# CrispyChillies/Image-Retrieval---Thesis-2026

Hardware: AMD Instinct MI355X
Metric: queries/sec (embed+top-10) over 1M x 1024 gallery (higher is better)
Workload: dtype f32 embed (two fp16 MFMA terms); bf16 MFMA candidates + f64 re-rank

## Files before the change

image-retrieval---thesis-2026_amd/csrc/k_conv3x3_d2h.hip:

```cpp
#include "mirx_kernels.h"

namespace mirx {

namespace {

typedef __attribute__((ext_vector_type(8))) _Float16 f16x8;
typedef __attribute__((ext_vector_type(16))) float f32x16;
typedef __attribute__((ext_vector_type(4))) unsigned u32x4;
typedef __attribute__((ext_vector_type(2))) float f32x2;
typedef __attribute__((ext_vector_type(2))) _Float16 f16x2;

#define LDS_PTR(p) ((__attribute__((address_space(3))) void *)(p))

constexpr int CIN = 128, COUT = 32;
constexpr int KC = 16;
constexpr int NST = CIN / KC;

template <int W, int R, int IPW = 1, int NW = 4>
__global__ __launch_bounds__(64 * NW, NW == 8 ? 1 : 2) void k_conv3x3_d2p(const uint16_t *__restrict__ yt, const uint16_t *__restrict__ w3,
                                                        const float *__restrict__ oscale, float *__restrict__ out,
                                                        int64_t out_bs, const float *__restrict__ in_inv,
                                                        unsigned *__restrict__ out_range, int64_t out_ps, int64_t n_img,
                                                        const float *__restrict__ pool_sc, const float *__restrict__ pool_sh,
                                                        float *__restrict__ pool_out, int64_t pool_bs) {
    constexpr int PW = W + 2, PR = R + 2;
    static_assert(IPW == 1 || R == W, "several images per workgroup: whole images only");
    constexpr int NPIX = IPW * PR * PW;
    constexpr int NP = (NPIX + 31) / 32;
    constexpr int PLANE = NP * 32 * 32;
    constexpr int STAGE = 2 * PLANE;
    constexpr int WSTAGE = 9 * 2 * COUT * KC * 2;
    constexpr int W_LDS0 = 2 * STAGE;
    constexpr int NOUT = IPW * R * W;
    constexpr int NBLK = (NOUT + 31) / 32;
    static_assert(NBLK <= 2 * NW, "two column blocks per wave");
    constexpr int PPW = (2 * NP + NW - 1) / NW;
    constexpr int WPW = (18 + NW - 1) / NW;
    extern __shared__ __attribute__((aligned(16))) char sm[];

    const int wave = __builtin_amdgcn_readfirstlane(threadIdx.x >> 6), lane = threadIdx.x & 63;
    const int half = lane >> 5, n = lane & 31;
    int strip = blockIdx.x;
    int64_t img = blockIdx.y;
    {
        const unsigned nstrip = gridDim.x, lin = blockIdx.x + nstrip * blockIdx.y, full = gridDim.y & ~7u;
        if (lin < nstrip * full) {
            const unsigned j = lin >> 3;
            strip = (int)(j % nstrip);
            img = (int64_t)(j / nstrip) * 8 + (lin & 7);
        }
    }
    const int oy0 = strip * R;
    constexpr unsigned IMG_BYTES = 16u * W * W * 32u;
    img *= IPW;
    const int n_here = (int)(n_img - img < IPW ? n_img - img : IPW);
    const __amdgpu_buffer_rsrc_t yrsrc = __builtin_amdgcn_make_buffer_rsrc((void *)(yt + img * (int64_t)(IMG_BYTES / 2)), 0,
                                                                           (unsigned)n_here * IMG_BYTES, 0x00020000);
    unsigned a_src[PPW];
    int a_dst[PPW];
#pragma unroll
    for (int i = 0; i < PPW; ++i) {
        const int q = wave + NW * i;
        const int term = q / NP, piece = q % NP;
        const int pix = piece * 32 + (lane >> 1);
        const int ji = pix / (PR * PW), prem = pix % (PR * PW);
        const int pr = prem / PW, pc = prem % PW;
        const int iy = oy0 - 1 + pr, ix = pc - 1;
        const bool inside = q < 2 * NP && pix < NPIX && iy >= 0 && iy < W && ix >= 0 && ix < W;
        const int chunk = (lane & 1) ^ ((pix >> 3) & 1);
        a_src[i] = inside ? (unsigned)(ji * IMG_BYTES + (term * W * W + iy * W + ix) * 32 + chunk * 16) : 0xfffffff0u;
        a_dst[i] = q < 2 * NP ? term * PLANE + piece * 1024 : -1;
    }
    auto dma_a = [&](int st, int buf) {
#pragma unroll
        for (int i = 0; i < PPW; ++i)
            if (a_dst[i] >= 0) {
                const unsigned v = a_src[i] == 0xfffffff0u ? a_src[i] : a_src[i] + (unsigned)st * (2u * W * W * 32u);
                __builtin_amdgcn_raw_ptr_buffer_load_lds(yrsrc, LDS_PTR(sm + buf * STAGE + a_dst[i]), 16, v, 0, 0, 0);
            }
    };

    int pbase[2];
    bool live_blk[2];
#pragma unroll
    for (int t = 0; t < 2; ++t) {
        const int blk = wave + NW * t;
        live_blk[t] = blk < NBLK;
        int p = blk * 32 + n;
        if (p >= NOUT) p = NOUT - 1;
        const int pj = p / (R * W), pq = p % (R * W);
        pbase[t] = pj * (PR * PW) + (pq / W) * PW + (pq % W);
    }
    const int a_off = n * 32 + ((half ^ ((n >> 3) & 1)) << 4);
    const __amdgpu_buffer_rsrc_t wrsrc = __builtin_amdgcn_make_buffer_rsrc((void *)w3, 0, NST * WSTAGE, 0x00020000);
    const int w_voff = (lane >> 1) * 32 + (((lane & 1) ^ ((lane >> 4) & 1)) << 4);
    auto dma_w = [&](int st, int buf) {
#pragma unroll
        for (int i = 0; i < WPW; ++i) {
            const int piece = wave + NW * i;
            if (piece < 18)
                __builtin_amdgcn_raw_ptr_buffer_load_lds(wrsrc, LDS_PTR(sm + W_LDS0 + buf * WSTAGE + piece * 1024), 16, w_voff,
                                                         st * WSTAGE + piece * 1024, 0, 0);
        }
    };

    f32x16 acc[2];
#pragma unroll
    for (int t = 0; t < 2; ++t)
#pragma unroll
        for (int r = 0; r < 16; ++r) acc[t][r] = 0.f;

#define MIRX_D2P_READA(DST, TAP)                                                                   \
    {                                                                                              \
        DST[0] = *reinterpret_cast<const f16x8 *>(wb + (2 * (TAP)) * 1024 + a_off);                \
        DST[1] = *reinterpret_cast<const f16x8 *>(wb + (2 * (TAP) + 1) * 1024 + a_off);            \
    }
#define MIRX_D2P_READB(DST, TAP, T)                                                                \
    {                                                                                              \
        const int pix_ = pbase[T] + ((TAP) / 3) * PW + (TAP) % 3;                                  \
        const char *pb_ = sb + pix_ * 32 + ((half ^ ((pix_ >> 3) & 1)) << 4);                      \
        DST[0] = *reinterpret_cast<const f16x8 *>(pb_);                                            \
        DST[1] = *reinterpret_cast<const f16x8 *>(pb_ + PLANE);                                    \
    }
#define MIRX_D2P_MFMA(T, A, B)                                                                     \
    {                                                                                              \
        f32x16 c_ = acc[T];                                                                        \
        c_ = __builtin_amdgcn_mfma_f32_32x32x16_f16(A[1], B[0], c_, 0, 0, 0);                      \
        c_ = __builtin_amdgcn_mfma_f32_32x32x16_f16(A[0], B[1], c_, 0, 0, 0);                      \
        c_ = __builtin_amdgcn_mfma_f32_32x32x16_f16(A[0], B[0], c_, 0, 0, 0);                      \
        acc[T] = c_;                                                                               \
    }
    const bool two = live_blk[1];
    dma_w(0, 0);
    dma_a(0, 0);
    for (int st = 0; st < NST; ++st) {
        const int cur = st & 1;
        asm volatile("s_waitcnt vmcnt(0)" ::: "memory");
        __syncthreads();
        if (st + 1 < NST) {
            dma_w(st + 1, cur ^ 1);
            dma_a(st + 1, cur ^ 1);
        }
        __builtin_amdgcn_sched_barrier(0);
        const char *sb = sm + cur * STAGE;
        const char *wb = sm + W_LDS0 + cur * WSTAGE;
        f16x8 a0[2], a1[2], b0[2], b1[2];
        MIRX_D2P_READA(a0, 0)
        MIRX_D2P_READB(b0, 0, 0)
        if (two) {
#pragma unroll
            for (int tap = 0; tap < 9; ++tap) {
                MIRX_D2P_READB(b1, tap, 1)
                if (tap + 1 < 9) {
                    if (tap & 1) { MIRX_D2P_READA(a0, tap + 1) } else { MIRX_D2P_READA(a1, tap + 1) }
                }
                __builtin_amdgcn_sched_barrier(0);
                if (tap & 1) { MIRX_D2P_MFMA(0, a1, b0) } else { MIRX_D2P_MFMA(0, a0, b0) }
                if (tap + 1 < 9) MIRX_D2P_READB(b0, tap + 1, 0)
                __builtin_amdgcn_sched_barrier(0);
                if (tap & 1) { MIRX_D2P_MFMA(1, a1, b1) } else { MIRX_D2P_MFMA(1, a0, b1) }
            }
        } else {
#pragma unroll
            for (int tap = 0; tap < 9; ++tap) {
                if (tap + 1 < 9) {
                    MIRX_D2P_READB(b1, tap + 1, 0)
                    if (tap & 1) { MIRX_D2P_READA(a0, tap + 1) } else { MIRX_D2P_READA(a1, tap + 1) }
                }
                __builtin_amdgcn_sched_barrier(0);
                if (tap & 1) { MIRX_D2P_MFMA(0, a1, b0) } else { MIRX_D2P_MFMA(0, a0, b0) }
#pragma unroll
                for (int q = 0; q < 2; ++q) b0[q] = b1[q];
            }
        }
    }
#undef MIRX_D2P_READA
#undef MIRX_D2P_READB
#undef MIRX_D2P_MFMA

    float *oi = out + img * out_bs + (int64_t)oy0 * W;
    float osc[16];
#pragma unroll
    for (int r = 0; r < 16; ++r) osc[r] = oscale[8 * (r >> 2) + (r & 3) + 4 * half];
    constexpr int ACT_PITCH = NOUT + 1;
    float *s_act = reinterpret_cast<float *>(sm);
    const bool pooled_twin = IPW == 1 && pool_out != nullptr;
    float psc[16], psh[16];
    if (pooled_twin) {
#pragma unroll
        for (int r = 0; r < 16; ++r) {
            psc[r] = pool_sc[8 * (r >> 2) + (r & 3) + 4 * half];
            psh[r] = pool_sh[8 * (r >> 2) + (r & 3) + 4 * half];
        }
        __syncthreads();
    }
#pragma unroll
    for (int t = 0; t < 2; ++t) {
        const int p = (wave + NW * t) * 32 + n;
        const int pj = p / (R * W), pq = p % (R * W);
        const bool live = live_blk[t] && p < NOUT && pj < n_here && oy0 + pq / W < W;
        const int pimg = (int)img + (pj < n_here ? pj : 0);
        float vmax = 0.f;
        if (live) {
            const float x_inv = in_inv[pimg];
            float *op = oi + (int64_t)pj * out_bs + pq;
#pragma unroll
            for (int r = 0; r < 16; ++r) {
                const int oc = 8 * (r >> 2) + (r & 3) + 4 * half;
                const float v = acc[t][r] * (osc[r] * x_inv);
                vmax = range_max(vmax, v);
                op[(int64_t)oc * out_ps] = v;
                if (pooled_twin) s_act[oc * ACT_PITCH + p] = fmaxf(fmaf(v, psc[r], psh[r]), 0.0f);
            }
        }
        if (out_range && live_blk[t]) {
            if (IPW == 1) range_publish(out_range, (int)img, vmax, lane);
            else range_publish_lanes(out_range, pimg, vmax, lane);
        }
    }
    if constexpr (IPW == 1) {
        if (pooled_twin) {
            __syncthreads();
            constexpr int W2 = W / 2, R2 = R / 2, NP2 = R2 * W2;
            static_assert(R % 2 == 0 && W % 2 == 0, "whole row pairs");
            const int rows_here = W - oy0 < R ? W - oy0 : R;
            float *po = pool_out + img * pool_bs + (int64_t)(oy0 / 2) * W2;
            for (int i = threadIdx.x; i < COUT * NP2; i += 64 * NW) {
                const int oc = i / NP2, q = i % NP2, py = q / W2, px = q % W2;
                if (2 * py < rows_here) {
                    const float *a = s_act + oc * ACT_PITCH + (2 * py) * W + 2 * px;
                    po[(int64_t)oc * (W2 * W2) + q] = (a[0] + a[1] + a[W] + a[W + 1]) * 0.25f;
                }
            }
        }
    }
}

template <int W, int R, int IPW = 1, int NW = 4>
hipError_t launch_d2p(const uint16_t *yt, const uint16_t *w2, const float *oscale, int64_t n, float *out, int64_t out_bs,
                      const float *in_inv, float *out_range, int64_t out_ps, hipStream_t st, const float *pool_sc = nullptr,
                      const float *pool_sh = nullptr, float *pool_out = nullptr, int64_t pool_bs = 0) {
    constexpr int NP = (IPW * (R + 2) * (W + 2) + 31) / 32;
    const size_t lds = (size_t)2 * 2 * NP * 1024 + 2 * 9 * 2 * 32 * 16 * 2;
    static_assert((size_t)2 * 2 * NP * 1024 + 2 * 9 * 2 * 32 * 16 * 2 <= 160 * 1024, "LDS of one CU");
    static unsigned long long attr_devs = 0;
    if (first_use_on_device(attr_devs)) {
        hipError_t e = hipFuncSetAttribute(reinterpret_cast<const void *>(k_conv3x3_d2p<W, R, IPW, NW>),
                                           hipFuncAttributeMaxDynamicSharedMemorySize, (int)lds);
        if (e != hipSuccess) return e;
    }
    hipLaunchKernelGGL((k_conv3x3_d2p<W, R, IPW, NW>), dim3((W + R - 1) / R, (unsigned)((n + IPW - 1) / IPW)), dim3(64 * NW), lds,
                       st, yt, w2, oscale, out, out_bs, in_inv, reinterpret_cast<unsigned *>(out_range), out_ps, n, pool_sc, pool_sh,
                       pool_out, pool_bs);
    return hipGetLastError();
}

}

bool conv3x3_takes_small(int64_t n, int side) {
    const int64_t wgs = side == 56 ? 14 * n : side == 28 ? 4 * n : side == 14 ? n : (n + 3) / 4;
    return wgs < conv3x3_small_max_wg();
}

hipError_t launch_conv3x3_d2p(const uint16_t *yt, const uint16_t *w2, const float *oscale, int64_t n, int side, float *out,
                              int64_t out_bs, const float *in_inv, float *out_range, int64_t out_ps, hipStream_t st,
                              const float *pool_sc, const float *pool_sh, float *pool_out, int64_t pool_bs) {
    if (n <= 0) return hipSuccess;
    if (n > 65535 || !in_inv || !oscale) return hipErrorInvalidValue;
    if (!out_ps) out_ps = (int64_t)side * side;
    if (out_ps < (int64_t)side * side) return hipErrorInvalidValue;
    if (pool_out && (!pool_sc || !pool_sh || side == 7 || pool_bs < (int64_t)COUT * (side / 2) * (side / 2)))
        return hipErrorInvalidValue;
    if (conv3x3_takes_small(n, side)) {
        if (pool_out) return hipErrorInvalidValue;
        return launch_conv3x3_d2s(yt, w2, oscale, n, side, out, out_bs, in_inv, out_range, out_ps, st);
    }
#ifndef MIRX_D2P_WAVES
#define MIRX_D2P_WAVES 4
#endif
#if MIRX_D2P_WAVES == 8
    if (pool_out) return hipErrorInvalidValue;
    if (side == 56) return launch_d2p<56, 8, 1, 8>(yt, w2, oscale, n, out, out_bs, in_inv, out_range, out_ps, st);
    if (side == 28) return launch_d2p<28, 14, 1, 8>(yt, w2, oscale, n, out, out_bs, in_inv, out_range, out_ps, st);
    if (side == 14) return launch_d2p<14, 14, 2, 8>(yt, w2, oscale, n, out, out_bs, in_inv, out_range, out_ps, st);
    if (side == 7) return launch_d2p<7, 7, 8, 8>(yt, w2, oscale, n, out, out_bs, in_inv, out_range, out_ps, st);
#else
    if (side == 56) return launch_d2p<56, 4>(yt, w2, oscale, n, out, out_bs, in_inv, out_range, out_ps, st, pool_sc, pool_sh, pool_out, pool_bs);
    if (side == 28) return launch_d2p<28, 8>(yt, w2, oscale, n, out, out_bs, in_inv, out_range, out_ps, st, pool_sc, pool_sh, pool_out, pool_bs);
    if (side == 14) return launch_d2p<14, 14>(yt, w2, oscale, n, out, out_bs, in_inv, out_range, out_ps, st, pool_sc, pool_sh, pool_out, pool_bs);
    if (side == 7) return launch_d2p<7, 7, 4>(yt, w2, oscale, n, out, out_bs, in_inv, out_range, out_ps, st);
#endif
    return hipErrorInvalidValue;
}

}
```

Measured before the change: 42710.

## Add flat pixel-tiled 3x3 conv kernel for 28 and 7 sides

Adds a new conv3x3 kernel that tiles the flattened batch-by-pixel space into fixed blocks of 32-pixel groups, so tiles may cross image boundaries. Out-of-image taps read from a zeroed LDS record instead of padding each image tile. Blocks are remapped across the grid in groups of eight, and the pooled twin output is computed from the tile. Sides 28 and 7 switch to it from the row-tiled kernel, which is meant to cut halo overhead and padding waste on small images. The cost is extra per-pixel offset arithmetic and more complex boundary handling.

```diff
diff --git a/image-retrieval---thesis-2026_amd/csrc/k_conv3x3_d2h.hip b/image-retrieval---thesis-2026_amd/csrc/k_conv3x3_d2h.hip
--- a/image-retrieval---thesis-2026_amd/csrc/k_conv3x3_d2h.hip
+++ b/image-retrieval---thesis-2026_amd/csrc/k_conv3x3_d2h.hip
@@ -236,6 +236,249 @@
     }
 }
 
+constexpr int d2t_blocks(int side) { return side == 28 ? 7 : 8; }
+constexpr int TW = 4;
+constexpr unsigned OOR = 0x80000000u;
+
+template <int W, int NB>
+__global__ __launch_bounds__(64 * TW, 2) void k_conv3x3_d2t(const uint16_t *__restrict__ yt, const uint16_t *__restrict__ w3,
+                                                        const float *__restrict__ oscale, float *__restrict__ out,
+                                                        int64_t out_bs, const float *__restrict__ in_inv,
+                                                        unsigned *__restrict__ out_range, int64_t out_ps, int64_t n_img,
+                                                        const float *__restrict__ pool_sc, const float *__restrict__ pool_sh,
+                                                        float *__restrict__ pool_out, int64_t pool_bs) {
+    constexpr int HW = W * W;
+    constexpr int NOUT = NB * 32;
+    constexpr int NPIX = NOUT + 2 * W + 2;
+    constexpr int ZREC = (NPIX + 7) & ~7;
+    constexpr int NP = (ZREC + 8 + 31) / 32;
+    constexpr int PLANE = NP * 32 * 32;
+    constexpr int STAGE = 2 * PLANE;
+    constexpr int WSTAGE = 9 * 2 * COUT * KC * 2;
+    constexpr int W_LDS0 = 2 * STAGE;
+    static_assert(NB <= 2 * TW, "two blocks per wave");
+    constexpr int PPW = (2 * NP + TW - 1) / TW;
+    constexpr int WPW = (18 + TW - 1) / TW;
+    constexpr unsigned IMG_BYTES = 16u * HW * 32u;
+    extern __shared__ __attribute__((aligned(16))) char sm[];
+
+    const int wave = __builtin_amdgcn_readfirstlane(threadIdx.x >> 6), lane = threadIdx.x & 63;
+    const int half = lane >> 5, n = lane & 31;
+    const int64_t total = n_img * HW;
+    unsigned tile = blockIdx.x;
+    {
+        const unsigned per = gridDim.x >> 3;
+        if (tile < per * 8) tile = (tile & 7) * per + (tile >> 3);
+    }
+    const int64_t p0 = (int64_t)tile * NOUT;
+    const int64_t s0 = p0 - (W + 1);
+    const int64_t slo = s0 < 0 ? 0 : s0, shi = s0 + NPIX < total ? s0 + NPIX : total;
+    const int64_t img0 = slo / HW;
+    const unsigned nimg = (unsigned)((shi - 1) / HW - img0 + 1);
+    const __amdgpu_buffer_rsrc_t yrsrc = __builtin_amdgcn_make_buffer_rsrc((void *)(yt + img0 * (int64_t)(IMG_BYTES / 2)), 0,
+                                                                           nimg * IMG_BYTES, 0x00020000);
+    unsigned a_src[PPW];
+    int a_dst[PPW];
+#pragma unroll
+    for (int i = 0; i < PPW; ++i) {
+        const int q = wave + TW * i;
+        const int term = q / NP, piece = q % NP;
+        const int r = piece * 32 + (lane >> 1);
+        const int64_t s = s0 + r;
+        const bool inside = q < 2 * NP && r < NPIX && s >= 0 && s < total;
+        const int chunk = (lane & 1) ^ ((r >> 3) & 1);
+        const int64_t si = inside ? s : img0 * HW;
+        a_src[i] = inside ? (unsigned)(si / HW - img0) * IMG_BYTES + (unsigned)((term * HW + si % HW) * 32 + chunk * 16) : OOR;
+        a_dst[i] = q < 2 * NP ? term * PLANE + piece * 1024 : -1;
+    }
+    auto dma_a = [&](int st, int buf) {
+#pragma unroll
+        for (int i = 0; i < PPW; ++i)
+            if (a_dst[i] >= 0)
+            {
+                const unsigned v = a_src[i] + (unsigned)st * (2u * W * W * 32u);
+                __builtin_amdgcn_raw_ptr_buffer_load_lds(yrsrc, LDS_PTR(sm + buf * STAGE + a_dst[i]), 16, v, 0, 0, 0);
+            }
+    };
+
+    int boff[2][9];
+    bool live_blk[2];
+#pragma unroll
+    for (int t = 0; t < 2; ++t) {
+        const int blk = wave + TW * t;
+        live_blk[t] = blk < NB;
+        const int pl = (blk < NB ? blk : NB - 1) * 32 + n;
+        const int q = (int)((p0 + pl) % HW), y = q / W, x = q % W;
+#pragma unroll
+        for (int tap = 0; tap < 9; ++tap) {
+            const int dy = tap / 3, dx = tap % 3;
+            const bool ok = y + dy - 1 >= 0 && y + dy - 1 < W && x + dx - 1 >= 0 && x + dx - 1 < W;
+            const int r = pl + dy * W + dx;
+            boff[t][tap] = (ok ? r : ZREC + (r & 7)) * 32 + ((half ^ ((r >> 3) & 1)) << 4);
+        }
+    }
+    const int a_off = n * 32 + ((half ^ ((n >> 3) & 1)) << 4);
+    const __amdgpu_buffer_rsrc_t wrsrc = __builtin_amdgcn_make_buffer_rsrc((void *)w3, 0, NST * WSTAGE, 0x00020000);
+    const int w_voff = (lane >> 1) * 32 + (((lane & 1) ^ ((lane >> 4) & 1)) << 4);
+    auto dma_w = [&](int st, int buf) {
+#pragma unroll
+        for (int i = 0; i < WPW; ++i) {
+            const int piece = wave + TW * i;
+            if (piece < 18)
+                __builtin_amdgcn_raw_ptr_buffer_load_lds(wrsrc, LDS_PTR(sm + W_LDS0 + buf * WSTAGE + piece * 1024), 16, w_voff,
+                                                         st * WSTAGE + piece * 1024, 0, 0);
+        }
+    };
+
+    f32x16 acc[2];
+#pragma unroll
+    for (int t = 0; t < 2; ++t)
+#pragma unroll
+        for (int r = 0; r < 16; ++r) acc[t][r] = 0.f;
+
+#define MIRX_D2T_READA(DST, TAP)                                                                   \
+    {                                                                                              \
+        DST[0] = *reinterpret_cast<const f16x8 *>(wb + (2 * (TAP)) * 1024 + a_off);                \
+        DST[1] = *reinterpret_cast<const f16x8 *>(wb + (2 * (TAP) + 1) * 1024 + a_off);            \
+    }
+#define MIRX_D2T_READB(DST, TAP, T)                                                                \
+    {                                                                                              \
+        const char *pb_ = sb + boff[T][TAP];                                                       \
+        DST[0] = *reinterpret_cast<const f16x8 *>(pb_);                                            \
+        DST[1] = *reinterpret_cast<const f16x8 *>(pb_ + PLANE);                                    \
+    }
+#define MIRX_D2T_MFMA(T, A, B)                                                                     \
+    {                                                                                              \
+        f32x16 c_ = acc[T];                                                                        \
+        c_ = __builtin_amdgcn_mfma_f32_32x32x16_f16(A[1], B[0], c_, 0, 0, 0);                      \
+        c_ = __builtin_amdgcn_mfma_f32_32x32x16_f16(A[0], B[1], c_, 0, 0, 0);                      \
+        c_ = __builtin_amdgcn_mfma_f32_32x32x16_f16(A[0], B[0], c_, 0, 0, 0);                      \
+        acc[T] = c_;                                                                               \
+    }
+    const bool two = live_blk[1];
+    dma_w(0, 0);
+    dma_a(0, 0);
+    for (int st = 0; st < NST; ++st) {
+        const int cur = st & 1;
+        asm volatile("s_waitcnt vmcnt(0)" ::: "memory");
+        __syncthreads();
+        if (st + 1 < NST) {
+            dma_w(st + 1, cur ^ 1);
+            dma_a(st + 1, cur ^ 1);
+        }
+        __builtin_amdgcn_sched_barrier(0);
+        const char *sb = sm + cur * STAGE;
+        const char *wb = sm + W_LDS0 + cur * WSTAGE;
+        f16x8 a0[2], a1[2], b0[2], b1[2];
+        MIRX_D2T_READA(a0, 0)
+        MIRX_D2T_READB(b0, 0, 0)
+        if (two) {
+#pragma unroll
+            for (int tap = 0; tap < 9; ++tap) {
+                MIRX_D2T_READB(b1, tap, 1)
+                if (tap + 1 < 9) {
+                    if (tap & 1) { MIRX_D2T_READA(a0, tap + 1) } else { MIRX_D2T_READA(a1, tap + 1) }
+                }
+                __builtin_amdgcn_sched_barrier(0);
+                if (tap & 1) { MIRX_D2T_MFMA(0, a1, b0) } else { MIRX_D2T_MFMA(0, a0, b0) }
+                if (tap + 1 < 9) MIRX_D2T_READB(b0, tap + 1, 0)
+                __builtin_amdgcn_sched_barrier(0);
+                if (tap & 1) { MIRX_D2T_MFMA(1, a1, b1) } else { MIRX_D2T_MFMA(1, a0, b1) }
+            }
+        } else {
+#pragma unroll
+            for (int tap = 0; tap < 9; ++tap) {
+                if (tap + 1 < 9) {
+                    MIRX_D2T_READB(b1, tap + 1, 0)
+                    if (tap & 1) { MIRX_D2T_READA(a0, tap + 1) } else { MIRX_D2T_READA(a1, tap + 1) }
+                }
+                __builtin_amdgcn_sched_barrier(0);
+                if (tap & 1) { MIRX_D2T_MFMA(0, a1, b0) } else { MIRX_D2T_MFMA(0, a0, b0) }
+#pragma unroll
+                for (int q = 0; q < 2; ++q) b0[q] = b1[q];
+            }
+        }
+    }
+#undef MIRX_D2T_READA
+#undef MIRX_D2T_READB
+#undef MIRX_D2T_MFMA
+
+    float osc[16];
+#pragma unroll
+    for (int r = 0; r < 16; ++r) osc[r] = oscale[8 * (r >> 2) + (r & 3) + 4 * half];
+    constexpr int ACT_PITCH = NOUT + 1;
+    static_assert(COUT * ACT_PITCH * 4 <= 2 * STAGE, "activations fit the stage buffers");
+    float *s_act = reinterpret_cast<float *>(sm);
+    const bool pooled_twin = W % 2 == 0 && pool_out != nullptr;
+    float psc[16], psh[16];
+    if (pooled_twin) {
+#pragma unroll
+        for (int r = 0; r < 16; ++r) {
+            psc[r] = pool_sc[8 * (r >> 2) + (r & 3) + 4 * half];
+            psh[r] = pool_sh[8 * (r >> 2) + (r & 3) + 4 * half];
+        }
+        __syncthreads();
+    }
+#pragma unroll
+    for (int t = 0; t < 2; ++t) {
+        const int pl = (wave + TW * t) * 32 + n;
+        const int64_t p = p0 + pl;
+        const bool live = live_blk[t] && p < total;
+        const int pimg = (int)((live ? p : total - 1) / HW);
+        float vmax = 0.f;
+        if (live) {
+            const float x_inv = in_inv[pimg];
+            float *op = out + pimg * out_bs + (int)(p - (int64_t)pimg * HW);
+#pragma unroll
+            for (int r = 0; r < 16; ++r) {
+                const int oc = 8 * (r >> 2) + (r & 3) + 4 * half;
+                const float v = acc[t][r] * (osc[r] * x_inv);
+                vmax = range_max(vmax, v);
+                op[(int64_t)oc * out_ps] = v;
+                if (pooled_twin) s_act[oc * ACT_PITCH + pl] = fmaxf(fmaf(v, psc[r], psh[r]), 0.0f);
+            }
+        }
+        if (out_range && live_blk[t]) {
+            if constexpr (HW % NOUT == 0) range_publish(out_range, pimg, vmax, lane);
+            else range_publish_lanes(out_range, pimg, vmax, lane);
+        }
+    }
+    if (pooled_twin) {
+        constexpr int W2 = W / 2, RP = 2 * W;
+        __syncthreads();
+        const int64_t pend = p0 + NOUT < total ? p0 + NOUT : total;
+        const int64_t k0 = (p0 + RP - 1) / RP;
+        const int nq = ((int)(pend / RP - k0) > 0 ? (int)(pend / RP - k0) : 0) * W2;
+        for (int i = threadIdx.x; i < COUT * nq; i += 64 * TW) {
+            const int oc = i / nq, j = i % nq, px = j % W2;
+            const int64_t k = k0 + j / W2, pimg = k / W2;
+            const int py = (int)(k % W2);
+            const float *a = s_act + oc * ACT_PITCH + (int)(k * RP - p0) + 2 * px;
+            pool_out[pimg * pool_bs + (int64_t)oc * (W2 * W2) + py * W2 + px] = (a[0] + a[1] + a[W] + a[W + 1]) * 0.25f;
+        }
+    }
+}
+
+template <int W, int NB = d2t_blocks(W)>
+hipError_t launch_d2t(const uint16_t *yt, const uint16_t *w2, const float *oscale, int64_t n, float *out, int64_t out_bs,
+                      const float *in_inv, float *out_range, int64_t out_ps, hipStream_t st, const float *pool_sc = nullptr,
+                      const float *pool_sh = nullptr, float *pool_out = nullptr, int64_t pool_bs = 0) {
+    static_assert(W % 2 || (NB * 32) % (2 * W) == 0, "the pooled twin needs whole row pairs in a tile");
+    constexpr int NP = (((NB * 32 + 2 * W + 2 + 7) & ~7) + 8 + 31) / 32;
+    constexpr size_t lds = (size_t)2 * 2 * NP * 1024 + 2 * 9 * 2 * 32 * 16 * 2;
+    static_assert(lds <= 80 * 1024, "two workgroups per CU");
+    static unsigned long long attr_devs = 0;
+    if (first_use_on_device(attr_devs)) {
+        hipError_t e = hipFuncSetAttribute(reinterpret_cast<const void *>(k_conv3x3_d2t<W, NB>),
+                                           hipFuncAttributeMaxDynamicSharedMemorySize, (int)lds);
+        if (e != hipSuccess) return e;
+    }
+    const int64_t ntile = (n * W * W + NB * 32 - 1) / (NB * 32);
+    hipLaunchKernelGGL((k_conv3x3_d2t<W, NB>), dim3((unsigned)ntile), dim3(64 * TW), lds, st, yt, w2, oscale, out, out_bs, in_inv,
+                       reinterpret_cast<unsigned *>(out_range), out_ps, n, pool_sc, pool_sh, pool_out, pool_bs);
+    return hipGetLastError();
+}
+
 template <int W, int R, int IPW = 1, int NW = 4>
 hipError_t launch_d2p(const uint16_t *yt, const uint16_t *w2, const float *oscale, int64_t n, float *out, int64_t out_bs,
                       const float *in_inv, float *out_range, int64_t out_ps, hipStream_t st, const float *pool_sc = nullptr,
@@ -258,7 +501,7 @@
 }
 
 bool conv3x3_takes_small(int64_t n, int side) {
-    const int64_t wgs = side == 56 ? 14 * n : side == 28 ? 4 * n : side == 14 ? n : (n + 3) / 4;
+    const int64_t wgs = side == 56 ? 14 * n : side == 14 ? n : (n * side * side + d2t_blocks(side) * 32 - 1) / (d2t_blocks(side) * 32);
     return wgs < conv3x3_small_max_wg();
 }
 
@@ -286,9 +529,9 @@
     if (side == 7) return launch_d2p<7, 7, 8, 8>(yt, w2, oscale, n, out, out_bs, in_inv, out_range, out_ps, st);
 #else
     if (side == 56) return launch_d2p<56, 4>(yt, w2, oscale, n, out, out_bs, in_inv, out_range, out_ps, st, pool_sc, pool_sh, pool_out, pool_bs);
-    if (side == 28) return launch_d2p<28, 8>(yt, w2, oscale, n, out, out_bs, in_inv, out_range, out_ps, st, pool_sc, pool_sh, pool_out, pool_bs);
+    if (side == 28) return launch_d2t<28>(yt, w2, oscale, n, out, out_bs, in_inv, out_range, out_ps, st, pool_sc, pool_sh, pool_out, pool_bs);
     if (side == 14) return launch_d2p<14, 14>(yt, w2, oscale, n, out, out_bs, in_inv, out_range, out_ps, st, pool_sc, pool_sh, pool_out, pool_bs);
-    if (side == 7) return launch_d2p<7, 7, 4>(yt, w2, oscale, n, out, out_bs, in_inv, out_range, out_ps, st);
+    if (side == 7) return launch_d2t<7>(yt, w2, oscale, n, out, out_bs, in_inv, out_range, out_ps, st);
 #endif
     return hipErrorInvalidValue;
 }
```

Result: no change. 42860, median of 6 (+0.4%).

## Drop column halo from conv3x3 LDS tile, redirect edge taps to zero records

Applied to the files above, without the earlier changes.

The staged input tile in LDS no longer holds the left and right padding columns. Each row is loaded contiguously, and out-of-image horizontal taps are redirected to 16 zero records placed behind the image. This reduces LDS footprint and DMA piece count per stage, and each tap's B-operand offset is precomputed once per thread. The unused 8-wave variant is removed. The trade-off is 18 extra registers per thread for the offset table and reliance on the zero tail records being written correctly.

```diff
diff --git a/image-retrieval---thesis-2026_amd/csrc/k_conv3x3_d2h.hip b/image-retrieval---thesis-2026_amd/csrc/k_conv3x3_d2h.hip
--- a/image-retrieval---thesis-2026_amd/csrc/k_conv3x3_d2h.hip
+++ b/image-retrieval---thesis-2026_amd/csrc/k_conv3x3_d2h.hip
@@ -16,20 +16,30 @@
 constexpr int KC = 16;
 constexpr int NST = CIN / KC;
 
-template <int W, int R, int IPW = 1, int NW = 4>
-__global__ __launch_bounds__(64 * NW, NW == 8 ? 1 : 2) void k_conv3x3_d2p(const uint16_t *__restrict__ yt, const uint16_t *__restrict__ w3,
-                                                        const float *__restrict__ oscale, float *__restrict__ out,
-                                                        int64_t out_bs, const float *__restrict__ in_inv,
-                                                        unsigned *__restrict__ out_range, int64_t out_ps, int64_t n_img,
-                                                        const float *__restrict__ pool_sc, const float *__restrict__ pool_sh,
-                                                        float *__restrict__ pool_out, int64_t pool_bs) {
-    constexpr int PW = W + 2, PR = R + 2;
+constexpr int D2P_NW = 4;
+constexpr int D2P_WSTAGE = 9 * 2 * COUT * KC * 2;
+
+template <int W, int R, int IPW>
+constexpr int d2p_pieces() { return (IPW * (R + 2) * W + 16 + 31) / 32; }
+template <int W, int R, int IPW>
+constexpr int d2p_lds_bytes() { return 2 * 2 * d2p_pieces<W, R, IPW>() * 1024 + 2 * D2P_WSTAGE; }
+
+template <int W, int R, int IPW = 1>
+__global__ __launch_bounds__(64 * D2P_NW, 2) void k_conv3x3_d2p(const uint16_t *__restrict__ yt, const uint16_t *__restrict__ w3,
+                                                       const float *__restrict__ oscale, float *__restrict__ out,
+                                                       int64_t out_bs, const float *__restrict__ in_inv,
+                                                       unsigned *__restrict__ out_range, int64_t out_ps, int64_t n_img,
+                                                       const float *__restrict__ pool_sc, const float *__restrict__ pool_sh,
+                                                       float *__restrict__ pool_out, int64_t pool_bs) {
+    constexpr int NW = D2P_NW;
+    constexpr int PR = R + 2;
     static_assert(IPW == 1 || R == W, "several images per workgroup: whole images only");
-    constexpr int NPIX = IPW * PR * PW;
-    constexpr int NP = (NPIX + 31) / 32;
+    constexpr int NPIX = IPW * PR * W;
+    constexpr int NP = d2p_pieces<W, R, IPW>();
+    static_assert(NP * 32 >= NPIX + 16, "16 zero records behind the image");
     constexpr int PLANE = NP * 32 * 32;
     constexpr int STAGE = 2 * PLANE;
-    constexpr int WSTAGE = 9 * 2 * COUT * KC * 2;
+    constexpr int WSTAGE = D2P_WSTAGE;
     constexpr int W_LDS0 = 2 * STAGE;
     constexpr int NOUT = IPW * R * W;
     constexpr int NBLK = (NOUT + 31) / 32;
@@ -63,12 +73,11 @@
         const int q = wave + NW * i;
         const int term = q / NP, piece = q % NP;
         const int pix = piece * 32 + (lane >> 1);
-        const int ji = pix / (PR * PW), prem = pix % (PR * PW);
-        const int pr = prem / PW, pc = prem % PW;
-        const int iy = oy0 - 1 + pr, ix = pc - 1;
-        const bool inside = q < 2 * NP && pix < NPIX && iy >= 0 && iy < W && ix >= 0 && ix < W;
+        const int ji = pix / (PR * W), prem = pix % (PR * W);
+        const int iy = oy0 - 1 + prem / W;
+        const bool inside = q < 2 * NP && pix < NPIX && iy >= 0 && iy < W;
         const int chunk = (lane & 1) ^ ((pix >> 3) & 1);
-        a_src[i] = inside ? (unsigned)(ji * IMG_BYTES + (term * W * W + iy * W + ix) * 32 + chunk * 16) : 0xfffffff0u;
+        a_src[i] = inside ? (unsigned)(ji * IMG_BYTES + (term * W * W + (oy0 - 1) * W + prem) * 32 + chunk * 16) : 0xfffffff0u;
         a_dst[i] = q < 2 * NP ? term * PLANE + piece * 1024 : -1;
     }
     auto dma_a = [&](int st, int buf) {
@@ -80,7 +89,7 @@
             }
     };
 
-    int pbase[2];
+    int b_off[2][9];
     bool live_blk[2];
 #pragma unroll
     for (int t = 0; t < 2; ++t) {
@@ -89,7 +98,14 @@
         int p = blk * 32 + n;
         if (p >= NOUT) p = NOUT - 1;
         const int pj = p / (R * W), pq = p % (R * W);
-        pbase[t] = pj * (PR * PW) + (pq / W) * PW + (pq % W);
+        const int ox = pq % W;
+#pragma unroll
+        for (int tap = 0; tap < 9; ++tap) {
+            const int dx = tap % 3;
+            int pix = pj * (PR * W) + pq + (tap / 3) * W + dx - 1;
+            if ((dx == 0 && ox == 0) || (dx == 2 && ox == W - 1)) pix = NPIX + ((pix - NPIX) & 15);
+            b_off[t][tap] = pix * 32 + ((half ^ ((pix >> 3) & 1)) << 4);
+        }
     }
     const int a_off = n * 32 + ((half ^ ((n >> 3) & 1)) << 4);
     const __amdgpu_buffer_rsrc_t wrsrc = __builtin_amdgcn_make_buffer_rsrc((void *)w3, 0, NST * WSTAGE, 0x00020000);
@@ -117,8 +133,7 @@
     }
 #define MIRX_D2P_READB(DST, TAP, T)                                                                \
     {                                                                                              \
-        const int pix_ = pbase[T] + ((TAP) / 3) * PW + (TAP) % 3;                                  \
-        const char *pb_ = sb + pix_ * 32 + ((half ^ ((pix_ >> 3) & 1)) << 4);                      \
+        const char *pb_ = sb + b_off[T][TAP];                                                      \
         DST[0] = *reinterpret_cast<const f16x8 *>(pb_);                                            \
         DST[1] = *reinterpret_cast<const f16x8 *>(pb_ + PLANE);                                    \
     }
@@ -236,20 +251,19 @@
     }
 }
 
-template <int W, int R, int IPW = 1, int NW = 4>
+template <int W, int R, int IPW = 1>
 hipError_t launch_d2p(const uint16_t *yt, const uint16_t *w2, const float *oscale, int64_t n, float *out, int64_t out_bs,
                       const float *in_inv, float *out_range, int64_t out_ps, hipStream_t st, const float *pool_sc = nullptr,
                       const float *pool_sh = nullptr, float *pool_out = nullptr, int64_t pool_bs = 0) {
-    constexpr int NP = (IPW * (R + 2) * (W + 2) + 31) / 32;
-    const size_t lds = (size_t)2 * 2 * NP * 1024 + 2 * 9 * 2 * 32 * 16 * 2;
-    static_assert((size_t)2 * 2 * NP * 1024 + 2 * 9 * 2 * 32 * 16 * 2 <= 160 * 1024, "LDS of one CU");
+    constexpr int lds = d2p_lds_bytes<W, R, IPW>();
+    static_assert(lds <= 160 * 1024 / 2, "__launch_bounds__(256, 2): two workgroups in the 160 KiB of a CU");
     static unsigned long long attr_devs = 0;
     if (first_use_on_device(attr_devs)) {
-        hipError_t e = hipFuncSetAttribute(reinterpret_cast<const void *>(k_conv3x3_d2p<W, R, IPW, NW>),
-                                           hipFuncAttributeMaxDynamicSharedMemorySize, (int)lds);
+        hipError_t e = hipFuncSetAttribute(reinterpret_cast<const void *>(k_conv3x3_d2p<W, R, IPW>),
+                                           hipFuncAttributeMaxDynamicSharedMemorySize, lds);
         if (e != hipSuccess) return e;
     }
-    hipLaunchKernelGGL((k_conv3x3_d2p<W, R, IPW, NW>), dim3((W + R - 1) / R, (unsigned)((n + IPW - 1) / IPW)), dim3(64 * NW), lds,
+    hipLaunchKernelGGL((k_conv3x3_d2p<W, R, IPW>), dim3((W + R - 1) / R, (unsigned)((n + IPW - 1) / IPW)), dim3(64 * D2P_NW), lds,
                        st, yt, w2, oscale, out, out_bs, in_inv, reinterpret_cast<unsigned *>(out_range), out_ps, n, pool_sc, pool_sh,
                        pool_out, pool_bs);
     return hipGetLastError();
@@ -275,21 +289,10 @@
         if (pool_out) return hipErrorInvalidValue;
         return launch_conv3x3_d2s(yt, w2, oscale, n, side, out, out_bs, in_inv, out_range, out_ps, st);
     }
-#ifndef MIRX_D2P_WAVES
-#define MIRX_D2P_WAVES 4
-#endif
-#if MIRX_D2P_WAVES == 8
-    if (pool_out) return hipErrorInvalidValue;
-    if (side == 56) return launch_d2p<56, 8, 1, 8>(yt, w2, oscale, n, out, out_bs, in_inv, out_range, out_ps, st);
-    if (side == 28) return launch_d2p<28, 14, 1, 8>(yt, w2, oscale, n, out, out_bs, in_inv, out_range, out_ps, st);
-    if (side == 14) return launch_d2p<14, 14, 2, 8>(yt, w2, oscale, n, out, out_bs, in_inv, out_range, out_ps, st);
-    if (side == 7) return launch_d2p<7, 7, 8, 8>(yt, w2, oscale, n, out, out_bs, in_inv, out_range, out_ps, st);
-#else
     if (side == 56) return launch_d2p<56, 4>(yt, w2, oscale, n, out, out_bs, in_inv, out_range, out_ps, st, pool_sc, pool_sh, pool_out, pool_bs);
     if (side == 28) return launch_d2p<28, 8>(yt, w2, oscale, n, out, out_bs, in_inv, out_range, out_ps, st, pool_sc, pool_sh, pool_out, pool_bs);
     if (side == 14) return launch_d2p<14, 14>(yt, w2, oscale, n, out, out_bs, in_inv, out_range, out_ps, st, pool_sc, pool_sh, pool_out, pool_bs);
     if (side == 7) return launch_d2p<7, 7, 4>(yt, w2, oscale, n, out, out_bs, in_inv, out_range, out_ps, st);
-#endif
     return hipErrorInvalidValue;
 }
 
```

Measured after the change: 44520 before, 44490 after (median of 6 runs). No clear change (-0.1%).
